# LPD-EPFL/ByzantineMomentum

Measured on AMD Instinct MI355X. Metric: aggregations/sec (Byzantine-robust GAR over n workers x d dims; achieved HBM GB/s per GAR in roofline/per_gar), higher is better.
Workload: dtype f32; 1 GPU; C2 colwise: median + trmean(f=5), n=25, total d=11173962; n_workers=25, f=5, d_total=11173962, d_per_gpu=11173962, byzantine_rows=distinct buffers, row_placement=one torch.empty per row (what a caller of the rules has), parallelism=single GPU, collectives=none

## Files before the change

### byzantinemomentum_amd/csrc/bm_common.h

```cpp
#pragma once
#include <hip/hip_runtime.h>
#include <stdint.h>
#include <utility>
#include "../../include/bm_gar.h"
#include "launch_plan.h"

namespace bm {

struct RowTable {
  const float* p[BM_MAX_ROWS];
  RowTable advanced(int64_t by) const {
    RowTable t = *this;
    advance(t.p, by);
    return t;
  }
};

static inline int hip_code(hipError_t e) { return e == hipSuccess ? 0 : -(int)e; }

#define BM_LAUNCH_CHECK()                      \
  do {                                         \
    hipError_t e__ = hipGetLastError();        \
    if (e__ != hipSuccess) return hip_code(e__); \
  } while (0)

template <int N>
struct MergeExchange {
  static constexpr int kMax = (N < 2) ? 1 : (N * 10);
  struct Table {
    short a[kMax];
    short b[kMax];
    int count;
  };
  static constexpr Table make() {
    Table t{};
    t.count = 0;
    if (N < 2) return t;
    int tt = 0;
    while ((1 << tt) < N) ++tt;
    for (int p = 1 << (tt - 1); p > 0; p /= 2) {
      int q = 1 << (tt - 1), r = 0, d = p;
      while (true) {
        for (int i = 0; i < N - d; ++i)
          if ((i & p) == r) {
            t.a[t.count] = (short)i;
            t.b[t.count] = (short)(i + d);
            ++t.count;
          }
        if (q == p) break;
        d = q - p;
        q /= 2;
        r = p;
      }
    }
    return t;
  }
  static constexpr Table table = make();
};

__device__ __forceinline__ void cmp_exchange(float& a, float& b) {
  float lo, hi;
  asm("v_min_f32 %0, %1, %2" : "=v"(lo) : "v"(a), "v"(b));
  asm("v_max_f32 %0, %1, %2" : "=v"(hi) : "v"(a), "v"(b));
  a = lo;
  b = hi;
}

template <int N, size_t... I>
__device__ __forceinline__ void sort_network_impl(float (&x)[N], std::index_sequence<I...>) {
  (cmp_exchange(x[MergeExchange<N>::table.a[I]], x[MergeExchange<N>::table.b[I]]), ...);
}

template <int N>
__device__ __forceinline__ void sort_network(float (&x)[N]) {
  if constexpr (N >= 2)
    sort_network_impl<N>(x, std::make_index_sequence<MergeExchange<N>::table.count>{});
}

__device__ __forceinline__ float div_small_int(float x, float m, float rm) {
  const float q = x * rm;
  const float r = __builtin_fmaf(-q, m, x);
  const float q1 = __builtin_fmaf(r, rm, q);
  return (q1 == q1) ? q1 : q;
}

template <int VEC>
struct VecLoad;
template <>
struct VecLoad<4> {
  using T = float __attribute__((ext_vector_type(4)));
};
template <>
struct VecLoad<2> {
  using T = float __attribute__((ext_vector_type(2)));
};
template <>
struct VecLoad<1> {
  using T = float;
};

template <int VEC>
__device__ __forceinline__ void load_stream(const float* p, float (&dst)[VEC]) {
  using T = typename VecLoad<VEC>::T;
  const T v = __builtin_nontemporal_load(reinterpret_cast<const T*>(p));
  if constexpr (VEC == 1) {
    dst[0] = v;
  } else {
#pragma unroll
    for (int c = 0; c < VEC; ++c) dst[c] = v[c];
  }
}

template <int VEC>
__device__ __forceinline__ void load_stream_off(const float* base, uint32_t byte_off, float (&dst)[VEC]) {
  load_stream<VEC>(reinterpret_cast<const float*>(reinterpret_cast<const char*>(base) + byte_off), dst);
}

template <int VEC>
__device__ __forceinline__ void store_stream_off(float* base, uint32_t byte_off, const float (&src)[VEC]);

template <int VEC>
__device__ __forceinline__ void store_stream(float* p, const float (&src)[VEC]) {
  using T = typename VecLoad<VEC>::T;
  T v;
  if constexpr (VEC == 1) {
    v = src[0];
  } else {
#pragma unroll
    for (int c = 0; c < VEC; ++c) v[c] = src[c];
  }
  __builtin_nontemporal_store(v, reinterpret_cast<T*>(p));
}

template <int VEC>
__device__ __forceinline__ void store_stream_off(float* base, uint32_t byte_off, const float (&src)[VEC]) {
  store_stream<VEC>(reinterpret_cast<float*>(reinterpret_cast<char*>(base) + byte_off), src);
}

template <int VEC>
__device__ __forceinline__ void store_result(float* p, const float (&src)[VEC]) {
  using T = typename VecLoad<VEC>::T;
  T v;
  if constexpr (VEC == 1) {
    v = src[0];
  } else {
#pragma unroll
    for (int c = 0; c < VEC; ++c) v[c] = src[c];
  }
  *reinterpret_cast<T*>(p) = v;
}
template <int VEC>
__device__ __forceinline__ void store_result_off(float* base, uint32_t byte_off, const float (&src)[VEC]) {
  store_result<VEC>(reinterpret_cast<float*>(reinterpret_cast<char*>(base) + byte_off), src);
}
template <int VEC>
__device__ __forceinline__ void store_result_policy(float* p, const float (&src)[VEC], int nt) {
  if (nt)
    store_stream<VEC>(p, src);
  else
    store_result<VEC>(p, src);
}

constexpr int kColMaxBlocks = 256 * 64;

static inline int lds_opt_in(const void* kernel, size_t dynamic_bytes, size_t static_bytes) {
  if (dynamic_bytes + static_bytes <= 48u * 1024u) return 0;
  return hip_code(hipFuncSetAttribute(kernel, hipFuncAttributeMaxDynamicSharedMemorySize, (int)dynamic_bytes));
}

static inline int compute_units() {
  static int cached[16] = {0};
  int dev = 0;
  if (hipGetDevice(&dev) != hipSuccess || dev < 0 || dev >= 16) dev = 0;
  if (cached[dev] == 0) {
    int cus = 0;
    if (hipDeviceGetAttribute(&cus, hipDeviceAttributeMultiprocessorCount, dev) != hipSuccess || cus <= 0) cus = 256;
    cached[dev] = cus;
  }
  return cached[dev];
}

__device__ __forceinline__ bool arrive_last(int* counter, int total, int* lds_flag) {
  asm volatile("s_waitcnt vmcnt(0)" ::: "memory");
  __syncthreads();
  if (threadIdx.x == 0) {
    __builtin_amdgcn_fence(__ATOMIC_RELEASE, "agent");
    asm volatile("s_waitcnt vmcnt(0)" ::: "memory");
    const int ticket = atomicAdd(counter, 1);
    const int last = (ticket == total - 1) ? 1 : 0;
    if (last) __builtin_amdgcn_fence(__ATOMIC_ACQUIRE, "agent");
    *lds_flag = last;
  }
  __syncthreads();
  return *lds_flag != 0;
}

__device__ __forceinline__ int32_t load_index_coherent(const int32_t* p) {
  return __hip_atomic_load(p, __ATOMIC_RELAXED, __HIP_MEMORY_SCOPE_AGENT);
}

template <int BLOCK>
__device__ __forceinline__ double block_reduce_sum(double v, double* lds ) {
#pragma unroll
  for (int off = 32; off > 0; off >>= 1) v += __shfl_down(v, off, 64);
  const int wave = threadIdx.x >> 6, lane = threadIdx.x & 63;
  if (lane == 0) lds[wave] = v;
  __syncthreads();
  double r = 0.0;
  if (threadIdx.x == 0) {
#pragma unroll
    for (int w = 0; w < BLOCK / 64; ++w) r += lds[w];
  }
  __syncthreads();
  return r;
}

__device__ __forceinline__ float byzantine_coordinate(float avg, float q, float fk, float scale, int attack_kind) {
  const float dir = ((attack_kind & 15) == BM_ATTACK_LITTLE) ? __builtin_sqrtf(q / (fk - 1.0f)) : -avg;
  const float att = dir * scale;
  return (attack_kind & BM_ATTACK_DIRECTION) ? att : avg + att;
}

}

namespace bm {
struct Tuning {
  int col_burst;
  int mean_burst;
  int step_burst;
  int step_stream;
  int pair_mode;
  int pair_planes;
  int pair_dither;
  double pair_tau;
  int study_burst;
  int step_stagger_us;
  int gram_steady;
  int bulyan_short;
  int pair_load_nt;
  int rank_algo;
  int col_wide;
  int brute_budget;
};
const Tuning& tuning();
Tuning& tuning_mutable();
}
```

### byzantinemomentum_amd/csrc/colwise_kernels.h

```cpp
#pragma once
#include "bm_common.h"

namespace bm {

constexpr int kColBlock = 256;

template <int N, int F>
__device__ __forceinline__ float trimmed_sum_static(const float (&x)[N]) {
  float t = 0.0f;
#pragma unroll
  for (int i = F; i < N - F; ++i) t += x[i];
  return t;
}

template <int N>
__device__ __forceinline__ float trimmed_sum(const float (&x)[N], int f) {
  float t = 0.0f;
  switch (f) {
#define BM_TRIM_CASE(F)                                             \
  case F:                                                           \
    if constexpr (2 * (F) < N) t = trimmed_sum_static<N, (F)>(x);   \
    break;
    BM_TRIM_CASE(0) BM_TRIM_CASE(1) BM_TRIM_CASE(2) BM_TRIM_CASE(3) BM_TRIM_CASE(4) BM_TRIM_CASE(5) BM_TRIM_CASE(6)
    BM_TRIM_CASE(7) BM_TRIM_CASE(8) BM_TRIM_CASE(9) BM_TRIM_CASE(10) BM_TRIM_CASE(11) BM_TRIM_CASE(12)
    BM_TRIM_CASE(13) BM_TRIM_CASE(14) BM_TRIM_CASE(15) BM_TRIM_CASE(16) BM_TRIM_CASE(17) BM_TRIM_CASE(18)
    BM_TRIM_CASE(19) BM_TRIM_CASE(20) BM_TRIM_CASE(21) BM_TRIM_CASE(22) BM_TRIM_CASE(23) BM_TRIM_CASE(24)
    BM_TRIM_CASE(25) BM_TRIM_CASE(26) BM_TRIM_CASE(27) BM_TRIM_CASE(28) BM_TRIM_CASE(29) BM_TRIM_CASE(30)
    BM_TRIM_CASE(31)
#undef BM_TRIM_CASE
    default:
      break;
  }
  return t;
}

template <int N, int F>
__device__ __forceinline__ float closest_sum_static(const float (&x)[N], float c) {
  constexpr int M = N - F;
  int s = 0;
#pragma unroll
  for (int t = 0; t < F; ++t) {
    const float dl = __builtin_fabsf(x[t] - c);
    const float dh = __builtin_fabsf(x[t + M] - c);
    s = (dl > dh) ? (t + 1) : s;
  }
  float w = 0.0f;
#pragma unroll
  for (int i = 0; i < N; ++i) {
    if (i < F)
      w += (i >= s) ? x[i] : 0.0f;
    else if (i >= M)
      w += (i < s + M) ? x[i] : 0.0f;
    else
      w += x[i];
  }
  return w;
}

template <int N>
__device__ __forceinline__ float closest_sum(const float (&x)[N], int f, float c) {
  float w = 0.0f;
  switch (f) {
#define BM_CLOSE_CASE(F)                                              \
  case F:                                                             \
    if constexpr (2 * (F) < N) w = closest_sum_static<N, (F)>(x, c);  \
    break;
    BM_CLOSE_CASE(0) BM_CLOSE_CASE(1) BM_CLOSE_CASE(2) BM_CLOSE_CASE(3) BM_CLOSE_CASE(4) BM_CLOSE_CASE(5) BM_CLOSE_CASE(6)
    BM_CLOSE_CASE(7) BM_CLOSE_CASE(8) BM_CLOSE_CASE(9) BM_CLOSE_CASE(10) BM_CLOSE_CASE(11) BM_CLOSE_CASE(12)
    BM_CLOSE_CASE(13) BM_CLOSE_CASE(14) BM_CLOSE_CASE(15) BM_CLOSE_CASE(16) BM_CLOSE_CASE(17) BM_CLOSE_CASE(18)
    BM_CLOSE_CASE(19) BM_CLOSE_CASE(20) BM_CLOSE_CASE(21) BM_CLOSE_CASE(22) BM_CLOSE_CASE(23) BM_CLOSE_CASE(24)
    BM_CLOSE_CASE(25) BM_CLOSE_CASE(26) BM_CLOSE_CASE(27) BM_CLOSE_CASE(28) BM_CLOSE_CASE(29) BM_CLOSE_CASE(30)
    BM_CLOSE_CASE(31)
#undef BM_CLOSE_CASE
    default:
      break;
  }
  return w;
}

template <int N, int OP, int STRIDE = kColBlock>
__device__ __forceinline__ float column_rule(float (&x)[N], int f, float inv_keep, float* ) {
  const float kNaN = __builtin_nanf("");
  const float kInf = __builtin_inff();
  bool has_nan = false;
#pragma unroll
  for (int i = 0; i < N; ++i) has_nan |= (x[i] != x[i]);

  if constexpr (OP == BM_OP_MEDIAN) {
    sort_network<N>(x);
    const float med = x[(N - 1) / 2];
    return has_nan ? kNaN : med;
  } else {
    int nan_count = 0;
    if (__builtin_amdgcn_ballot_w64(has_nan) != 0ull) {
#pragma unroll
      for (int i = 0; i < N; ++i) {
        const bool isn = (x[i] != x[i]);
        nan_count += isn ? 1 : 0;
        x[i] = isn ? kInf : x[i];
      }
    }
    sort_network<N>(x);
    float tsum = 0.0f;
    if constexpr (OP == BM_OP_TRMEAN || OP == BM_OP_PHOCAS) tsum = trimmed_sum<N>(x, f);
    if constexpr (OP == BM_OP_TRMEAN) {
      const float r = div_small_int(tsum, (float)(N - 2 * f), inv_keep);
      return (nan_count > f) ? kNaN : r;
    } else {
      float c;
      if constexpr (OP == BM_OP_PHOCAS) {
        c = div_small_int(tsum, (float)(N - 2 * f), 1.0f / (float)(N - 2 * f));
        if (nan_count > f) c = kNaN;
      } else {
        c = has_nan ? kNaN : x[(N - 1) / 2];
      }
      const int m = N - f;
      const float wsum = closest_sum<N>(x, f, c);
      const float r = div_small_int(wsum, (float)m, inv_keep);
      return (c != c || nan_count > f) ? kNaN : r;
    }
  }
}

template <int N, int OP, int VEC, bool ABLATE_STORE = false>
__global__ __launch_bounds__(kColBlock) void colwise_kernel(RowTable rows, int64_t nvec, int tail,
                                                            int f, float inv_keep, int nt_result,
                                                            float* __restrict__ out) {
  float* const lds = nullptr;
  const uint32_t nv = (uint32_t)nvec;
  const uint32_t stride = gridDim.x * kColBlock;
  for (uint32_t v = blockIdx.x * kColBlock + threadIdx.x; v < nv; v += stride) {
    const uint32_t off = v * (uint32_t)(VEC * sizeof(float));
    float x[VEC][N];
#pragma unroll
    for (int i = 0; i < N; ++i) {
      float t[VEC];
      load_stream_off<VEC>(rows.p[i], off, t);
#pragma unroll
      for (int c = 0; c < VEC; ++c) x[c][i] = t[c];
    }
    float r[VEC];
#pragma unroll
    for (int c = 0; c < VEC; ++c) r[c] = column_rule<N, OP>(x[c], f, inv_keep, lds);
    if constexpr (ABLATE_STORE) {
      if (r[0] == 1.2345678e-30f) store_stream_off<VEC>(out, off, r);
    } else if (nt_result) {
      store_stream_off<VEC>(out, off, r);
    } else {
      store_result_off<VEC>(out, off, r);
    }
  }
  if (VEC > 1 && blockIdx.x == gridDim.x - 1 && (int)threadIdx.x < tail) {
    const int64_t j = nvec * VEC + threadIdx.x;
    float x[N];
#pragma unroll
    for (int i = 0; i < N; ++i) x[i] = rows.p[i][j];
    out[j] = column_rule<N, OP>(x, f, inv_keep, lds);
  }
}

constexpr int kBurstThreads = 1024;
constexpr int kBurstLdsBytes = 160 * 1024;

template <int N, int OP, int VEC>
__global__ __launch_bounds__(kBurstThreads) void colwise_burst_kernel(RowTable rows, int64_t nvec, int tail, int f,
                                                                      float inv_keep, float* __restrict__ out) {
  using V = typename VecLoad<VEC>::T;
  constexpr int kSlots = kBurstLdsBytes / (kBurstThreads * VEC * (int)sizeof(float));
  __shared__ V stage[kSlots * kBurstThreads];
  const uint32_t nv = (uint32_t)nvec, tid = threadIdx.x;
  const uint32_t span = gridDim.x * kBurstThreads;
  const uint32_t iters = (nv + span - 1) / span;
  const uint32_t first = blockIdx.x * kBurstThreads + tid;
  for (uint32_t p0 = 0; p0 < iters; p0 += kSlots) {
    const uint32_t p1 = (p0 + kSlots < iters) ? p0 + kSlots : iters;
    for (uint32_t it = p0; it < p1; ++it) {
      const uint32_t v = it * span + first;
      if (v < nv) {
        const uint32_t off = v * (uint32_t)(VEC * sizeof(float));
        float x[VEC][N];
#pragma unroll
        for (int i = 0; i < N; ++i) {
          float t[VEC];
          load_stream_off<VEC>(rows.p[i], off, t);
#pragma unroll
          for (int c = 0; c < VEC; ++c) x[c][i] = t[c];
        }
        float r[VEC];
#pragma unroll
        for (int c = 0; c < VEC; ++c) r[c] = column_rule<N, OP>(x[c], f, inv_keep, nullptr);
        V packed;
        if constexpr (VEC == 1) {
          packed = r[0];
        } else {
#pragma unroll
          for (int c = 0; c < VEC; ++c) packed[c] = r[c];
        }
        stage[(it - p0) * kBurstThreads + tid] = packed;
      }
    }
    __syncthreads();
    for (uint32_t it = p0; it < p1; ++it) {
      const uint32_t v = it * span + first;
      if (v < nv) {
        const uint32_t off = v * (uint32_t)(VEC * sizeof(float));
        const V packed = stage[(it - p0) * kBurstThreads + tid];
        __builtin_nontemporal_store(packed, reinterpret_cast<V*>(reinterpret_cast<char*>(out) + off));
      }
    }
  }
  if (VEC > 1 && blockIdx.x == gridDim.x - 1 && (int)tid < tail) {
    const int64_t j = nvec * VEC + tid;
    float x[N];
#pragma unroll
    for (int i = 0; i < N; ++i) x[i] = rows.p[i][j];
    out[j] = column_rule<N, OP>(x, f, inv_keep, nullptr);
  }
}

constexpr int kEvalMaxBlocks = 2048;
constexpr Caps kEvalCaps = caps_of(kEvalMaxBlocks);

constexpr int kEvalFinishThreads = 1024;
template <int THREADS>
__global__ __launch_bounds__(THREADS) void eval_finish_kernel(const double* __restrict__ partial, int nparts,
                                                                         double* __restrict__ out) {
  __shared__ double red[THREADS / 64];
  double tot = 0.0;
  for (int b = threadIdx.x; b < nparts; b += THREADS) tot += partial[b];
  const double r = block_reduce_sum<THREADS>(tot, red);
  if (threadIdx.x == 0) out[0] = r;
}


}
```

Before: 5307 agg/s.

## Use min3/med3/max3 sorting networks and compile-time trim count for trmean

Replaces the Batcher merge-exchange sorting network with precomputed tables that mix 3-element sorts (v_min3/v_med3/v_max3) with 2-element compare-exchanges, which cuts the instruction count of the per-column sort for n up to 25. It also dispatches the runtime trim count f to a compile-time constant for trmean, so trimmed sums and the NaN handling specialise fully. The aim is to lower ALU cost in the column-wise median and trmean kernels, at the price of more template instantiations and code size. The hand-built tables must be correct sorting networks.

```diff
diff --git a/byzantinemomentum_amd/csrc/bm_common.h b/byzantinemomentum_amd/csrc/bm_common.h
--- a/byzantinemomentum_amd/csrc/bm_common.h
+++ b/byzantinemomentum_amd/csrc/bm_common.h
@@ -4,6 +4,7 @@
 #include <utility>
 #include "../../include/bm_gar.h"
 #include "launch_plan.h"
+#include "sort_tables.h"
 
 namespace bm {
 
@@ -66,14 +67,39 @@
   b = hi;
 }
 
+__device__ __forceinline__ void sort3(float& a, float& b, float& c) {
+  float lo, mid, hi;
+  asm("v_min3_f32 %0, %1, %2, %3" : "=v"(lo) : "v"(a), "v"(b), "v"(c));
+  asm("v_med3_f32 %0, %1, %2, %3" : "=v"(mid) : "v"(a), "v"(b), "v"(c));
+  asm("v_max3_f32 %0, %1, %2, %3" : "=v"(hi) : "v"(a), "v"(b), "v"(c));
+  a = lo;
+  b = mid;
+  c = hi;
+}
+
 template <int N, size_t... I>
 __device__ __forceinline__ void sort_network_impl(float (&x)[N], std::index_sequence<I...>) {
   (cmp_exchange(x[MergeExchange<N>::table.a[I]], x[MergeExchange<N>::table.b[I]]), ...);
 }
 
+template <int N, size_t I>
+__device__ __forceinline__ void sort_table_op(float (&x)[N]) {
+  constexpr SortOp op = SortTable<N>::ops[I];
+  if constexpr (op.c < 0)
+    cmp_exchange(x[op.a], x[op.b]);
+  else
+    sort3(x[op.a], x[op.b], x[op.c]);
+}
+template <int N, size_t... I>
+__device__ __forceinline__ void sort_table_impl(float (&x)[N], std::index_sequence<I...>) {
+  (sort_table_op<N, I>(x), ...);
+}
+
 template <int N>
 __device__ __forceinline__ void sort_network(float (&x)[N]) {
-  if constexpr (N >= 2)
+  if constexpr (N >= 2 && N <= kSortTableMaxRows)
+    sort_table_impl<N>(x, std::make_index_sequence<SortTable<N>::count>{});
+  else if constexpr (N >= 2)
     sort_network_impl<N>(x, std::make_index_sequence<MergeExchange<N>::table.count>{});
 }
 
diff --git a/byzantinemomentum_amd/csrc/colwise_kernels.h b/byzantinemomentum_amd/csrc/colwise_kernels.h
--- a/byzantinemomentum_amd/csrc/colwise_kernels.h
+++ b/byzantinemomentum_amd/csrc/colwise_kernels.h
@@ -122,6 +122,59 @@
   }
 }
 
+constexpr int kTrimSortMaxRows = kSortTableMaxRows;
+template <int N, int F>
+__device__ __forceinline__ float trmean_column_static(float (&x)[N], float inv_keep) {
+  const float kNaN = __builtin_nanf("");
+  const float kInf = __builtin_inff();
+  bool has_nan = false;
+#pragma unroll
+  for (int i = 0; i < N; ++i) has_nan |= (x[i] != x[i]);
+  int nan_count = 0;
+  if (__builtin_amdgcn_ballot_w64(has_nan) != 0ull) {
+#pragma unroll
+    for (int i = 0; i < N; ++i) {
+      const bool isn = (x[i] != x[i]);
+      nan_count += isn ? 1 : 0;
+      x[i] = isn ? kInf : x[i];
+    }
+  }
+  sort_network<N>(x);
+  const float r = div_small_int(trimmed_sum_static<N, F>(x), (float)(N - 2 * F), inv_keep);
+  return (nan_count > F) ? kNaN : r;
+}
+
+template <int N, int OP, typename Body>
+__device__ __forceinline__ void with_trim_count(int f, Body&& body) {
+  if constexpr (OP == BM_OP_TRMEAN && N <= kTrimSortMaxRows) {
+    static_assert(kTrimSortMaxRows <= 26, "cases for f = 0 .. 12");
+    switch (f) {
+#define BM_TRIM_CASE(F)                                                       \
+  case F:                                                                     \
+    if constexpr (2 * (F) < N) body(std::integral_constant<int, (F)>{});      \
+    break;
+      BM_TRIM_CASE(0) BM_TRIM_CASE(1) BM_TRIM_CASE(2) BM_TRIM_CASE(3) BM_TRIM_CASE(4) BM_TRIM_CASE(5) BM_TRIM_CASE(6)
+      BM_TRIM_CASE(7) BM_TRIM_CASE(8) BM_TRIM_CASE(9) BM_TRIM_CASE(10) BM_TRIM_CASE(11) BM_TRIM_CASE(12)
+#undef BM_TRIM_CASE
+      default:
+        break;
+    }
+  } else {
+    body(std::integral_constant<int, -1>{});
+  }
+}
+
+template <int N, int OP, int VEC, int F>
+__device__ __forceinline__ void column_rules(float (&x)[VEC][N], int f, float inv_keep, float (&r)[VEC]) {
+#pragma unroll
+  for (int c = 0; c < VEC; ++c) {
+    if constexpr (F >= 0)
+      r[c] = trmean_column_static<N, F>(x[c], inv_keep);
+    else
+      r[c] = column_rule<N, OP>(x[c], f, inv_keep, nullptr);
+  }
+}
+
 template <int N, int OP, int VEC, bool ABLATE_STORE = false>
 __global__ __launch_bounds__(kColBlock) void colwise_kernel(RowTable rows, int64_t nvec, int tail,
                                                             int f, float inv_keep, int nt_result,
@@ -129,27 +182,29 @@
   float* const lds = nullptr;
   const uint32_t nv = (uint32_t)nvec;
   const uint32_t stride = gridDim.x * kColBlock;
-  for (uint32_t v = blockIdx.x * kColBlock + threadIdx.x; v < nv; v += stride) {
-    const uint32_t off = v * (uint32_t)(VEC * sizeof(float));
-    float x[VEC][N];
-#pragma unroll
-    for (int i = 0; i < N; ++i) {
-      float t[VEC];
-      load_stream_off<VEC>(rows.p[i], off, t);
-#pragma unroll
-      for (int c = 0; c < VEC; ++c) x[c][i] = t[c];
-    }
-    float r[VEC];
-#pragma unroll
-    for (int c = 0; c < VEC; ++c) r[c] = column_rule<N, OP>(x[c], f, inv_keep, lds);
-    if constexpr (ABLATE_STORE) {
-      if (r[0] == 1.2345678e-30f) store_stream_off<VEC>(out, off, r);
-    } else if (nt_result) {
-      store_stream_off<VEC>(out, off, r);
-    } else {
-      store_result_off<VEC>(out, off, r);
-    }
-  }
+  with_trim_count<N, OP>(f, [&](auto trim) {
+    constexpr int F = decltype(trim)::value;
+    for (uint32_t v = blockIdx.x * kColBlock + threadIdx.x; v < nv; v += stride) {
+      const uint32_t off = v * (uint32_t)(VEC * sizeof(float));
+      float x[VEC][N];
+#pragma unroll
+      for (int i = 0; i < N; ++i) {
+        float t[VEC];
+        load_stream_off<VEC>(rows.p[i], off, t);
+#pragma unroll
+        for (int c = 0; c < VEC; ++c) x[c][i] = t[c];
+      }
+      float r[VEC];
+      column_rules<N, OP, VEC, F>(x, f, inv_keep, r);
+      if constexpr (ABLATE_STORE) {
+        if (r[0] == 1.2345678e-30f) store_stream_off<VEC>(out, off, r);
+      } else if (nt_result) {
+        store_stream_off<VEC>(out, off, r);
+      } else {
+        store_result_off<VEC>(out, off, r);
+      }
+    }
+  });
   if (VEC > 1 && blockIdx.x == gridDim.x - 1 && (int)threadIdx.x < tail) {
     const int64_t j = nvec * VEC + threadIdx.x;
     float x[N];
@@ -172,43 +227,45 @@
   const uint32_t span = gridDim.x * kBurstThreads;
   const uint32_t iters = (nv + span - 1) / span;
   const uint32_t first = blockIdx.x * kBurstThreads + tid;
-  for (uint32_t p0 = 0; p0 < iters; p0 += kSlots) {
-    const uint32_t p1 = (p0 + kSlots < iters) ? p0 + kSlots : iters;
-    for (uint32_t it = p0; it < p1; ++it) {
-      const uint32_t v = it * span + first;
-      if (v < nv) {
-        const uint32_t off = v * (uint32_t)(VEC * sizeof(float));
-        float x[VEC][N];
-#pragma unroll
-        for (int i = 0; i < N; ++i) {
-          float t[VEC];
-          load_stream_off<VEC>(rows.p[i], off, t);
-#pragma unroll
-          for (int c = 0; c < VEC; ++c) x[c][i] = t[c];
+  with_trim_count<N, OP>(f, [&](auto trim) {
+    constexpr int F = decltype(trim)::value;
+    for (uint32_t p0 = 0; p0 < iters; p0 += kSlots) {
+      const uint32_t p1 = (p0 + kSlots < iters) ? p0 + kSlots : iters;
+      for (uint32_t it = p0; it < p1; ++it) {
+        const uint32_t v = it * span + first;
+        if (v < nv) {
+          const uint32_t off = v * (uint32_t)(VEC * sizeof(float));
+          float x[VEC][N];
+#pragma unroll
+          for (int i = 0; i < N; ++i) {
+            float t[VEC];
+            load_stream_off<VEC>(rows.p[i], off, t);
+#pragma unroll
+            for (int c = 0; c < VEC; ++c) x[c][i] = t[c];
+          }
+          float r[VEC];
+          column_rules<N, OP, VEC, F>(x, f, inv_keep, r);
+          V packed;
+          if constexpr (VEC == 1) {
+            packed = r[0];
+          } else {
+#pragma unroll
+            for (int c = 0; c < VEC; ++c) packed[c] = r[c];
+          }
+          stage[(it - p0) * kBurstThreads + tid] = packed;
         }
-        float r[VEC];
-#pragma unroll
-        for (int c = 0; c < VEC; ++c) r[c] = column_rule<N, OP>(x[c], f, inv_keep, nullptr);
-        V packed;
-        if constexpr (VEC == 1) {
-          packed = r[0];
-        } else {
-#pragma unroll
-          for (int c = 0; c < VEC; ++c) packed[c] = r[c];
+      }
+      __syncthreads();
+      for (uint32_t it = p0; it < p1; ++it) {
+        const uint32_t v = it * span + first;
+        if (v < nv) {
+          const uint32_t off = v * (uint32_t)(VEC * sizeof(float));
+          const V packed = stage[(it - p0) * kBurstThreads + tid];
+          __builtin_nontemporal_store(packed, reinterpret_cast<V*>(reinterpret_cast<char*>(out) + off));
         }
-        stage[(it - p0) * kBurstThreads + tid] = packed;
-      }
-    }
-    __syncthreads();
-    for (uint32_t it = p0; it < p1; ++it) {
-      const uint32_t v = it * span + first;
-      if (v < nv) {
-        const uint32_t off = v * (uint32_t)(VEC * sizeof(float));
-        const V packed = stage[(it - p0) * kBurstThreads + tid];
-        __builtin_nontemporal_store(packed, reinterpret_cast<V*>(reinterpret_cast<char*>(out) + off));
-      }
-    }
-  }
+      }
+    }
+  });
   if (VEC > 1 && blockIdx.x == gridDim.x - 1 && (int)tid < tail) {
     const int64_t j = nvec * VEC + tid;
     float x[N];
diff --git a/byzantinemomentum_amd/csrc/sort_tables.h b/byzantinemomentum_amd/csrc/sort_tables.h
--- /dev/null
+++ b/byzantinemomentum_amd/csrc/sort_tables.h
@@ -0,0 +1,331 @@
+#pragma once
+
+namespace bm {
+
+struct SortOp {
+  signed char a, b, c;
+};
+
+constexpr int kSortTableMaxRows = 25;
+
+template <int N>
+struct SortTable;
+
+template <>
+struct SortTable<2> {
+  static constexpr int count = 1;
+  static constexpr SortOp ops[1] = {
+      {0, 1, -1},
+  };
+};
+
+template <>
+struct SortTable<3> {
+  static constexpr int count = 1;
+  static constexpr SortOp ops[1] = {
+      {0, 1, 2},
+  };
+};
+
+template <>
+struct SortTable<4> {
+  static constexpr int count = 4;
+  static constexpr SortOp ops[4] = {
+      {0, 1, 2}, {1, 3, -1}, {0, 1, -1}, {2, 3, -1},
+  };
+};
+
+template <>
+struct SortTable<5> {
+  static constexpr int count = 7;
+  static constexpr SortOp ops[7] = {
+      {0, 2, 4}, {1, 3, -1}, {0, 1, -1}, {2, 3, -1}, {1, 4, -1}, {1, 2, -1}, {3, 4, -1},
+  };
+};
+
+template <>
+struct SortTable<6> {
+  static constexpr int count = 8;
+  static constexpr SortOp ops[8] = {
+      {0, 2, 4}, {1, 3, 5}, {0, 1, -1}, {2, 3, -1}, {4, 5, -1}, {1, 4, -1}, {1, 2, -1}, {3, 4, -1},
+  };
+};
+
+template <>
+struct SortTable<7> {
+  static constexpr int count = 13;
+  static constexpr SortOp ops[13] = {
+      {0, 2, 4}, {1, 3, 5}, {2, 6, -1}, {0, 2, -1}, {4, 6, -1}, {0, 1, -1}, {2, 3, -1}, {4, 5, -1},
+      {1, 4, -1}, {3, 6, -1}, {1, 2, -1}, {3, 4, -1}, {5, 6, -1},
+  };
+};
+
+template <>
+struct SortTable<8> {
+  static constexpr int count = 17;
+  static constexpr SortOp ops[17] = {
+      {0, 2, 4}, {1, 3, 5}, {2, 6, -1}, {3, 7, -1}, {0, 2, -1}, {1, 3, -1}, {4, 6, -1}, {5, 7, -1},
+      {0, 1, -1}, {2, 3, -1}, {4, 5, -1}, {6, 7, -1}, {1, 4, -1}, {3, 6, -1}, {1, 2, -1}, {3, 4, -1},
+      {5, 6, -1},
+  };
+};
+
+template <>
+struct SortTable<9> {
+  static constexpr int count = 13;
+  static constexpr SortOp ops[13] = {
+      {0, 3, 6}, {1, 4, 7}, {2, 5, 8}, {0, 1, 2}, {3, 4, 5}, {6, 7, 8}, {2, 6, -1}, {1, 3, -1},
+      {4, 6, -1}, {5, 7, -1}, {2, 4, -1}, {2, 3, -1}, {5, 6, -1},
+  };
+};
+
+template <>
+struct SortTable<10> {
+  static constexpr int count = 22;
+  static constexpr SortOp ops[22] = {
+      {0, 3, 6}, {1, 4, 7}, {2, 5, 8}, {0, 1, 2}, {3, 4, 5}, {6, 7, 8}, {1, 9, -1}, {2, 6, -1},
+      {5, 9, -1}, {1, 3, -1}, {4, 6, -1}, {5, 7, -1}, {2, 4, -1}, {3, 5, -1}, {7, 9, -1}, {0, 1, -1},
+      {2, 3, -1}, {4, 5, -1}, {6, 7, -1}, {8, 9, -1}, {3, 4, -1}, {5, 6, -1},
+  };
+};
+
+template <>
+struct SortTable<11> {
+  static constexpr int count = 29;
+  static constexpr SortOp ops[29] = {
+      {0, 4, 8}, {1, 5, 9}, {2, 6, 10}, {0, 1, 2}, {4, 5, 6}, {8, 9, 10}, {3, 7, -1}, {1, 3, -1},
+      {5, 7, -1}, {2, 8, -1}, {3, 9, -1}, {2, 4, -1}, {3, 5, -1}, {6, 8, -1}, {7, 9, -1}, {0, 1, -1},
+      {2, 3, -1}, {4, 5, -1}, {6, 7, -1}, {8, 9, -1}, {1, 4, -1}, {3, 6, -1}, {5, 8, -1}, {7, 10, -1},
+      {1, 2, -1}, {3, 4, -1}, {5, 6, -1}, {7, 8, -1}, {9, 10, -1},
+  };
+};
+
+template <>
+struct SortTable<12> {
+  static constexpr int count = 31;
+  static constexpr SortOp ops[31] = {
+      {0, 4, 8}, {1, 5, 9}, {2, 6, 10}, {3, 7, 11}, {0, 1, 2}, {4, 5, 6}, {8, 9, 10}, {1, 3, -1},
+      {5, 7, -1}, {9, 11, -1}, {2, 8, -1}, {3, 9, -1}, {2, 4, -1}, {3, 5, -1}, {6, 8, -1}, {7, 9, -1},
+      {0, 1, -1}, {2, 3, -1}, {4, 5, -1}, {6, 7, -1}, {8, 9, -1}, {10, 11, -1}, {1, 4, -1}, {3, 6, -1},
+      {5, 8, -1}, {7, 10, -1}, {1, 2, -1}, {3, 4, -1}, {5, 6, -1}, {7, 8, -1}, {9, 10, -1},
+  };
+};
+
+template <>
+struct SortTable<13> {
+  static constexpr int count = 38;
+  static constexpr SortOp ops[38] = {
+      {0, 4, 8}, {1, 5, 9}, {2, 6, 10}, {3, 7, 11}, {0, 1, 2}, {4, 5, 6}, {8, 9, 10}, {4, 12, -1},
+      {0, 4, -1}, {8, 12, -1}, {1, 3, -1}, {5, 7, -1}, {9, 11, -1}, {2, 8, -1}, {3, 9, -1}, {6, 12, -1},
+      {2, 4, -1}, {3, 5, -1}, {6, 8, -1}, {7, 9, -1}, {10, 12, -1}, {0, 1, -1}, {2, 3, -1}, {4, 5, -1},
+      {6, 7, -1}, {8, 9, -1}, {10, 11, -1}, {1, 4, -1}, {3, 6, -1}, {5, 8, -1}, {7, 10, -1}, {9, 12, -1},
+      {1, 2, -1}, {3, 4, -1}, {5, 6, -1}, {7, 8, -1}, {9, 10, -1}, {11, 12, -1},
+  };
+};
+
+template <>
+struct SortTable<14> {
+  static constexpr int count = 44;
+  static constexpr SortOp ops[44] = {
+      {0, 4, 8}, {1, 5, 9}, {2, 6, 10}, {3, 7, 11}, {0, 1, 2}, {4, 5, 6}, {8, 9, 10}, {4, 12, -1},
+      {5, 13, -1}, {0, 4, -1}, {1, 5, -1}, {8, 12, -1}, {9, 13, -1}, {1, 3, -1}, {5, 7, -1}, {9, 11, -1},
+      {2, 8, -1}, {3, 9, -1}, {6, 12, -1}, {7, 13, -1}, {2, 4, -1}, {3, 5, -1}, {6, 8, -1}, {7, 9, -1},
+      {10, 12, -1}, {11, 13, -1}, {0, 1, -1}, {2, 3, -1}, {4, 5, -1}, {6, 7, -1}, {8, 9, -1}, {10, 11, -1},
+      {12, 13, -1}, {1, 4, -1}, {3, 6, -1}, {5, 8, -1}, {7, 10, -1}, {9, 12, -1}, {1, 2, -1}, {3, 4, -1},
+      {5, 6, -1}, {7, 8, -1}, {9, 10, -1}, {11, 12, -1},
+  };
+};
+
+template <>
+struct SortTable<15> {
+  static constexpr int count = 50;
+  static constexpr SortOp ops[50] = {
+      {0, 4, 8}, {1, 5, 9}, {2, 6, 10}, {3, 7, 11}, {0, 1, 2}, {4, 5, 6}, {8, 9, 10}, {12, 13, 14},
+      {4, 12, -1}, {5, 13, -1}, {6, 14, -1}, {0, 4, -1}, {1, 5, -1}, {2, 6, -1}, {8, 12, -1}, {9, 13, -1},
+      {10, 14, -1}, {1, 3, -1}, {5, 7, -1}, {9, 11, -1}, {2, 8, -1}, {3, 9, -1}, {6, 12, -1}, {7, 13, -1},
+      {2, 4, -1}, {3, 5, -1}, {6, 8, -1}, {7, 9, -1}, {10, 12, -1}, {11, 13, -1}, {0, 1, -1}, {2, 3, -1},
+      {4, 5, -1}, {6, 7, -1}, {8, 9, -1}, {10, 11, -1}, {12, 13, -1}, {1, 4, -1}, {3, 6, -1}, {5, 8, -1},
+      {7, 10, -1}, {9, 12, -1}, {11, 14, -1}, {1, 2, -1}, {3, 4, -1}, {5, 6, -1}, {7, 8, -1}, {9, 10, -1},
+      {11, 12, -1}, {13, 14, -1},
+  };
+};
+
+template <>
+struct SortTable<16> {
+  static constexpr int count = 55;
+  static constexpr SortOp ops[55] = {
+      {0, 4, 8}, {1, 5, 9}, {2, 6, 10}, {3, 7, 11}, {0, 1, 2}, {4, 5, 6}, {8, 9, 10}, {12, 13, 14},
+      {4, 12, -1}, {5, 13, -1}, {6, 14, -1}, {7, 15, -1}, {0, 4, -1}, {1, 5, -1}, {2, 6, -1}, {3, 7, -1},
+      {8, 12, -1}, {9, 13, -1}, {10, 14, -1}, {11, 15, -1}, {1, 3, -1}, {5, 7, -1}, {9, 11, -1}, {13, 15, -1},
+      {2, 8, -1}, {3, 9, -1}, {6, 12, -1}, {7, 13, -1}, {2, 4, -1}, {3, 5, -1}, {6, 8, -1}, {7, 9, -1},
+      {10, 12, -1}, {11, 13, -1}, {0, 1, -1}, {2, 3, -1}, {4, 5, -1}, {6, 7, -1}, {8, 9, -1}, {10, 11, -1},
+      {12, 13, -1}, {14, 15, -1}, {1, 4, -1}, {3, 6, -1}, {5, 8, -1}, {7, 10, -1}, {9, 12, -1}, {11, 14, -1},
+      {1, 2, -1}, {3, 4, -1}, {5, 6, -1}, {7, 8, -1}, {9, 10, -1}, {11, 12, -1}, {13, 14, -1},
+  };
+};
+
+template <>
+struct SortTable<17> {
+  static constexpr int count = 58;
+  static constexpr SortOp ops[58] = {
+      {0, 6, 12}, {1, 7, 13}, {2, 8, 14}, {3, 9, 15}, {4, 10, 16}, {0, 2, 4}, {1, 3, 5}, {6, 8, 10},
+      {7, 9, 11}, {12, 14, 16}, {4, 12, -1}, {5, 13, -1}, {2, 6, -1}, {3, 7, -1}, {8, 12, -1}, {9, 13, -1},
+      {10, 14, -1}, {11, 15, -1}, {4, 8, -1}, {5, 9, -1}, {7, 11, -1}, {1, 3, -1}, {4, 6, -1}, {5, 7, -1},
+      {9, 11, -1}, {13, 15, -1}, {7, 9, -1}, {10, 12, -1}, {11, 13, -1}, {0, 1, -1}, {2, 3, -1}, {4, 5, -1},
+      {6, 7, -1}, {8, 9, -1}, {10, 11, -1}, {12, 13, -1}, {14, 15, -1}, {1, 16, -1}, {1, 8, -1}, {3, 10, -1},
+      {5, 12, -1}, {7, 14, -1}, {9, 16, -1}, {1, 4, -1}, {3, 6, -1}, {5, 8, -1}, {7, 10, -1}, {9, 12, -1},
+      {11, 14, -1}, {13, 16, -1}, {1, 2, -1}, {3, 4, -1}, {5, 6, -1}, {7, 8, -1}, {9, 10, -1}, {11, 12, -1},
+      {13, 14, -1}, {15, 16, -1},
+  };
+};
+
+template <>
+struct SortTable<18> {
+  static constexpr int count = 56;
+  static constexpr SortOp ops[56] = {
+      {0, 6, 12}, {1, 7, 13}, {2, 8, 14}, {3, 9, 15}, {4, 10, 16}, {5, 11, 17}, {0, 2, 4}, {1, 3, 5},
+      {6, 8, 10}, {7, 9, 11}, {12, 14, 16}, {13, 15, 17}, {4, 12, -1}, {5, 13, -1}, {2, 6, -1}, {3, 7, -1},
+      {8, 12, -1}, {9, 13, -1}, {10, 14, -1}, {11, 15, -1}, {4, 8, -1}, {5, 9, -1}, {4, 6, -1}, {5, 7, -1},
+      {10, 12, -1}, {11, 13, -1}, {0, 1, -1}, {2, 3, -1}, {4, 5, -1}, {6, 7, -1}, {8, 9, -1}, {10, 11, -1},
+      {12, 13, -1}, {14, 15, -1}, {16, 17, -1}, {1, 16, -1}, {1, 8, -1}, {3, 10, -1}, {5, 12, -1}, {7, 14, -1},
+      {9, 16, -1}, {1, 4, -1}, {3, 6, -1}, {5, 8, -1}, {7, 10, -1}, {9, 12, -1}, {11, 14, -1}, {13, 16, -1},
+      {1, 2, -1}, {3, 4, -1}, {5, 6, -1}, {7, 8, -1}, {9, 10, -1}, {11, 12, -1}, {13, 14, -1}, {15, 16, -1},
+  };
+};
+
+template <>
+struct SortTable<19> {
+  static constexpr int count = 69;
+  static constexpr SortOp ops[69] = {
+      {0, 6, 12}, {1, 7, 13}, {2, 8, 14}, {3, 9, 15}, {4, 10, 16}, {5, 11, 17}, {0, 2, 4}, {1, 3, 5},
+      {6, 8, 10}, {7, 9, 11}, {12, 14, 16}, {13, 15, 17}, {2, 18, -1}, {4, 12, -1}, {5, 13, -1}, {10, 18, -1},
+      {2, 6, -1}, {3, 7, -1}, {8, 12, -1}, {9, 13, -1}, {10, 14, -1}, {11, 15, -1}, {4, 8, -1}, {5, 9, -1},
+      {6, 10, -1}, {14, 18, -1}, {0, 2, -1}, {4, 6, -1}, {5, 7, -1}, {8, 10, -1}, {12, 14, -1}, {16, 18, -1},
+      {6, 8, -1}, {10, 12, -1}, {11, 13, -1}, {0, 1, -1}, {2, 3, -1}, {4, 5, -1}, {6, 7, -1}, {8, 9, -1},
+      {10, 11, -1}, {12, 13, -1}, {14, 15, -1}, {16, 17, -1}, {1, 16, -1}, {3, 18, -1}, {1, 8, -1}, {3, 10, -1},
+      {5, 12, -1}, {7, 14, -1}, {9, 16, -1}, {11, 18, -1}, {1, 4, -1}, {3, 6, -1}, {5, 8, -1}, {7, 10, -1},
+      {9, 12, -1}, {11, 14, -1}, {13, 16, -1}, {15, 18, -1}, {1, 2, -1}, {3, 4, -1}, {5, 6, -1}, {7, 8, -1},
+      {9, 10, -1}, {11, 12, -1}, {13, 14, -1}, {15, 16, -1}, {17, 18, -1},
+  };
+};
+
+template <>
+struct SortTable<20> {
+  static constexpr int count = 79;
+  static constexpr SortOp ops[79] = {
+      {0, 6, 12}, {1, 7, 13}, {2, 8, 14}, {3, 9, 15}, {4, 10, 16}, {5, 11, 17}, {0, 2, 4}, {1, 3, 5},
+      {6, 8, 10}, {7, 9, 11}, {12, 14, 16}, {13, 15, 17}, {2, 18, -1}, {3, 19, -1}, {4, 12, -1}, {5, 13, -1},
+      {10, 18, -1}, {11, 19, -1}, {2, 6, -1}, {3, 7, -1}, {8, 12, -1}, {9, 13, -1}, {10, 14, -1}, {11, 15, -1},
+      {4, 8, -1}, {5, 9, -1}, {6, 10, -1}, {7, 11, -1}, {14, 18, -1}, {15, 19, -1}, {0, 2, -1}, {1, 3, -1},
+      {4, 6, -1}, {5, 7, -1}, {8, 10, -1}, {9, 11, -1}, {12, 14, -1}, {13, 15, -1}, {16, 18, -1}, {17, 19, -1},
+      {6, 8, -1}, {7, 9, -1}, {10, 12, -1}, {11, 13, -1}, {0, 1, -1}, {2, 3, -1}, {4, 5, -1}, {6, 7, -1},
+      {8, 9, -1}, {10, 11, -1}, {12, 13, -1}, {14, 15, -1}, {16, 17, -1}, {18, 19, -1}, {1, 16, -1}, {3, 18, -1},
+      {1, 8, -1}, {3, 10, -1}, {5, 12, -1}, {7, 14, -1}, {9, 16, -1}, {11, 18, -1}, {1, 4, -1}, {3, 6, -1},
+      {5, 8, -1}, {7, 10, -1}, {9, 12, -1}, {11, 14, -1}, {13, 16, -1}, {15, 18, -1}, {1, 2, -1}, {3, 4, -1},
+      {5, 6, -1}, {7, 8, -1}, {9, 10, -1}, {11, 12, -1}, {13, 14, -1}, {15, 16, -1}, {17, 18, -1},
+  };
+};
+
+template <>
+struct SortTable<21> {
+  static constexpr int count = 92;
+  static constexpr SortOp ops[92] = {
+      {0, 6, 12}, {1, 7, 13}, {2, 8, 14}, {3, 9, 15}, {4, 10, 16}, {5, 11, 17}, {0, 2, 4}, {1, 3, 5},
+      {6, 8, 10}, {7, 9, 11}, {12, 14, 16}, {13, 15, 17}, {2, 18, -1}, {3, 19, -1}, {4, 20, -1}, {4, 12, -1},
+      {5, 13, -1}, {10, 18, -1}, {11, 19, -1}, {12, 20, -1}, {0, 4, -1}, {2, 6, -1}, {3, 7, -1}, {8, 12, -1},
+      {9, 13, -1}, {10, 14, -1}, {11, 15, -1}, {16, 20, -1}, {4, 8, -1}, {5, 9, -1}, {6, 10, -1}, {7, 11, -1},
+      {12, 16, -1}, {14, 18, -1}, {15, 19, -1}, {0, 2, -1}, {1, 3, -1}, {4, 6, -1}, {5, 7, -1}, {8, 10, -1},
+      {9, 11, -1}, {12, 14, -1}, {13, 15, -1}, {16, 18, -1}, {17, 19, -1}, {10, 16, -1}, {2, 4, -1}, {6, 8, -1},
+      {7, 9, -1}, {10, 12, -1}, {11, 13, -1}, {14, 16, -1}, {18, 20, -1}, {0, 1, -1}, {2, 3, -1}, {4, 5, -1},
+      {6, 7, -1}, {8, 9, -1}, {10, 11, -1}, {12, 13, -1}, {14, 15, -1}, {16, 17, -1}, {18, 19, -1}, {1, 16, -1},
+      {3, 18, -1}, {5, 20, -1}, {1, 8, -1}, {3, 10, -1}, {5, 12, -1}, {7, 14, -1}, {9, 16, -1}, {11, 18, -1},
+      {13, 20, -1}, {1, 4, -1}, {3, 6, -1}, {5, 8, -1}, {7, 10, -1}, {9, 12, -1}, {11, 14, -1}, {13, 16, -1},
+      {15, 18, -1}, {17, 20, -1}, {1, 2, -1}, {3, 4, -1}, {5, 6, -1}, {7, 8, -1}, {9, 10, -1}, {11, 12, -1},
+      {13, 14, -1}, {15, 16, -1}, {17, 18, -1}, {19, 20, -1},
+  };
+};
+
+template <>
+struct SortTable<22> {
+  static constexpr int count = 98;
+  static constexpr SortOp ops[98] = {
+      {0, 8, 16}, {1, 9, 17}, {2, 10, 18}, {3, 11, 19}, {4, 12, 20}, {5, 13, 21}, {0, 2, 4}, {1, 3, 5},
+      {8, 10, 12}, {9, 11, 13}, {16, 18, 20}, {17, 19, 21}, {6, 14, -1}, {7, 15, -1}, {2, 6, -1}, {3, 7, -1},
+      {10, 14, -1}, {11, 15, -1}, {4, 16, -1}, {5, 17, -1}, {6, 18, -1}, {7, 19, -1}, {4, 8, -1}, {5, 9, -1},
+      {6, 10, -1}, {7, 11, -1}, {12, 16, -1}, {13, 17, -1}, {14, 18, -1}, {15, 19, -1}, {0, 2, -1}, {1, 3, -1},
+      {4, 6, -1}, {5, 7, -1}, {8, 10, -1}, {9, 11, -1}, {12, 14, -1}, {13, 15, -1}, {16, 18, -1}, {17, 19, -1},
+      {2, 8, -1}, {3, 9, -1}, {6, 12, -1}, {7, 13, -1}, {10, 16, -1}, {11, 17, -1}, {14, 20, -1}, {15, 21, -1},
+      {2, 4, -1}, {3, 5, -1}, {6, 8, -1}, {7, 9, -1}, {10, 12, -1}, {11, 13, -1}, {14, 16, -1}, {15, 17, -1},
+      {18, 20, -1}, {19, 21, -1}, {0, 1, -1}, {2, 3, -1}, {4, 5, -1}, {6, 7, -1}, {8, 9, -1}, {10, 11, -1},
+      {12, 13, -1}, {14, 15, -1}, {16, 17, -1}, {18, 19, -1}, {20, 21, -1}, {1, 16, -1}, {3, 18, -1}, {5, 20, -1},
+      {1, 8, -1}, {3, 10, -1}, {5, 12, -1}, {7, 14, -1}, {9, 16, -1}, {11, 18, -1}, {13, 20, -1}, {1, 4, -1},
+      {3, 6, -1}, {5, 8, -1}, {7, 10, -1}, {9, 12, -1}, {11, 14, -1}, {13, 16, -1}, {15, 18, -1}, {17, 20, -1},
+      {1, 2, -1}, {3, 4, -1}, {5, 6, -1}, {7, 8, -1}, {9, 10, -1}, {11, 12, -1}, {13, 14, -1}, {15, 16, -1},
+      {17, 18, -1}, {19, 20, -1},
+  };
+};
+
+template <>
+struct SortTable<23> {
+  static constexpr int count = 104;
+  static constexpr SortOp ops[104] = {
+      {0, 8, 16}, {1, 9, 17}, {2, 10, 18}, {3, 11, 19}, {4, 12, 20}, {5, 13, 21}, {6, 14, 22}, {0, 2, 4},
+      {1, 3, 5}, {8, 10, 12}, {9, 11, 13}, {16, 18, 20}, {17, 19, 21}, {7, 15, -1}, {2, 6, -1}, {3, 7, -1},
+      {10, 14, -1}, {11, 15, -1}, {18, 22, -1}, {4, 16, -1}, {5, 17, -1}, {6, 18, -1}, {7, 19, -1}, {4, 8, -1},
+      {5, 9, -1}, {6, 10, -1}, {7, 11, -1}, {12, 16, -1}, {13, 17, -1}, {14, 18, -1}, {15, 19, -1}, {0, 2, -1},
+      {1, 3, -1}, {4, 6, -1}, {5, 7, -1}, {8, 10, -1}, {9, 11, -1}, {12, 14, -1}, {13, 15, -1}, {16, 18, -1},
+      {17, 19, -1}, {20, 22, -1}, {2, 8, -1}, {3, 9, -1}, {6, 12, -1}, {7, 13, -1}, {10, 16, -1}, {11, 17, -1},
+      {14, 20, -1}, {15, 21, -1}, {2, 4, -1}, {3, 5, -1}, {6, 8, -1}, {7, 9, -1}, {10, 12, -1}, {11, 13, -1},
+      {14, 16, -1}, {15, 17, -1}, {18, 20, -1}, {19, 21, -1}, {0, 1, -1}, {2, 3, -1}, {4, 5, -1}, {6, 7, -1},
+      {8, 9, -1}, {10, 11, -1}, {12, 13, -1}, {14, 15, -1}, {16, 17, -1}, {18, 19, -1}, {20, 21, -1}, {1, 16, -1},
+      {3, 18, -1}, {5, 20, -1}, {7, 22, -1}, {1, 8, -1}, {3, 10, -1}, {5, 12, -1}, {7, 14, -1}, {9, 16, -1},
+      {11, 18, -1}, {13, 20, -1}, {15, 22, -1}, {1, 4, -1}, {3, 6, -1}, {5, 8, -1}, {7, 10, -1}, {9, 12, -1},
+      {11, 14, -1}, {13, 16, -1}, {15, 18, -1}, {17, 20, -1}, {19, 22, -1}, {1, 2, -1}, {3, 4, -1}, {5, 6, -1},
+      {7, 8, -1}, {9, 10, -1}, {11, 12, -1}, {13, 14, -1}, {15, 16, -1}, {17, 18, -1}, {19, 20, -1}, {21, 22, -1},
+  };
+};
+
+template <>
+struct SortTable<24> {
+  static constexpr int count = 107;
+  static constexpr SortOp ops[107] = {
+      {0, 8, 16}, {1, 9, 17}, {2, 10, 18}, {3, 11, 19}, {4, 12, 20}, {5, 13, 21}, {6, 14, 22}, {7, 15, 23},
+      {0, 2, 4}, {1, 3, 5}, {8, 10, 12}, {9, 11, 13}, {16, 18, 20}, {17, 19, 21}, {2, 6, -1}, {3, 7, -1},
+      {10, 14, -1}, {11, 15, -1}, {18, 22, -1}, {19, 23, -1}, {4, 16, -1}, {5, 17, -1}, {6, 18, -1}, {7, 19, -1},
+      {4, 8, -1}, {5, 9, -1}, {6, 10, -1}, {7, 11, -1}, {12, 16, -1}, {13, 17, -1}, {14, 18, -1}, {15, 19, -1},
+      {0, 2, -1}, {1, 3, -1}, {4, 6, -1}, {5, 7, -1}, {8, 10, -1}, {9, 11, -1}, {12, 14, -1}, {13, 15, -1},
+      {16, 18, -1}, {17, 19, -1}, {20, 22, -1}, {21, 23, -1}, {2, 8, -1}, {3, 9, -1}, {6, 12, -1}, {7, 13, -1},
+      {10, 16, -1}, {11, 17, -1}, {14, 20, -1}, {15, 21, -1}, {2, 4, -1}, {3, 5, -1}, {6, 8, -1}, {7, 9, -1},
+      {10, 12, -1}, {11, 13, -1}, {14, 16, -1}, {15, 17, -1}, {18, 20, -1}, {19, 21, -1}, {0, 1, -1}, {2, 3, -1},
+      {4, 5, -1}, {6, 7, -1}, {8, 9, -1}, {10, 11, -1}, {12, 13, -1}, {14, 15, -1}, {16, 17, -1}, {18, 19, -1},
+      {20, 21, -1}, {22, 23, -1}, {1, 16, -1}, {3, 18, -1}, {5, 20, -1}, {7, 22, -1}, {1, 8, -1}, {3, 10, -1},
+      {5, 12, -1}, {7, 14, -1}, {9, 16, -1}, {11, 18, -1}, {13, 20, -1}, {15, 22, -1}, {1, 4, -1}, {3, 6, -1},
+      {5, 8, -1}, {7, 10, -1}, {9, 12, -1}, {11, 14, -1}, {13, 16, -1}, {15, 18, -1}, {17, 20, -1}, {19, 22, -1},
+      {1, 2, -1}, {3, 4, -1}, {5, 6, -1}, {7, 8, -1}, {9, 10, -1}, {11, 12, -1}, {13, 14, -1}, {15, 16, -1},
+      {17, 18, -1}, {19, 20, -1}, {21, 22, -1},
+  };
+};
+
+template <>
+struct SortTable<25> {
+  static constexpr int count = 118;
+  static constexpr SortOp ops[118] = {
+      {0, 8, 16}, {1, 9, 17}, {2, 10, 18}, {3, 11, 19}, {4, 12, 20}, {5, 13, 21}, {6, 14, 22}, {7, 15, 23},
+      {0, 2, 4}, {1, 3, 5}, {8, 10, 12}, {9, 11, 13}, {16, 18, 20}, {17, 19, 21}, {8, 24, -1}, {0, 8, -1},
+      {16, 24, -1}, {2, 6, -1}, {3, 7, -1}, {10, 14, -1}, {11, 15, -1}, {18, 22, -1}, {19, 23, -1}, {4, 16, -1},
+      {5, 17, -1}, {6, 18, -1}, {7, 19, -1}, {12, 24, -1}, {4, 8, -1}, {5, 9, -1}, {6, 10, -1}, {7, 11, -1},
+      {12, 16, -1}, {13, 17, -1}, {14, 18, -1}, {15, 19, -1}, {20, 24, -1}, {0, 2, -1}, {1, 3, -1}, {4, 6, -1},
+      {5, 7, -1}, {8, 10, -1}, {9, 11, -1}, {12, 14, -1}, {13, 15, -1}, {16, 18, -1}, {17, 19, -1}, {20, 22, -1},
+      {21, 23, -1}, {2, 8, -1}, {3, 9, -1}, {6, 12, -1}, {7, 13, -1}, {10, 16, -1}, {11, 17, -1}, {14, 20, -1},
+      {15, 21, -1}, {18, 24, -1}, {2, 4, -1}, {3, 5, -1}, {6, 8, -1}, {7, 9, -1}, {10, 12, -1}, {11, 13, -1},
+      {14, 16, -1}, {15, 17, -1}, {18, 20, -1}, {19, 21, -1}, {22, 24, -1}, {0, 1, -1}, {2, 3, -1}, {4, 5, -1},
+      {6, 7, -1}, {8, 9, -1}, {10, 11, -1}, {12, 13, -1}, {14, 15, -1}, {16, 17, -1}, {18, 19, -1}, {20, 21, -1},
+      {22, 23, -1}, {1, 16, -1}, {3, 18, -1}, {5, 20, -1}, {7, 22, -1}, {9, 24, -1}, {1, 8, -1}, {3, 10, -1},
+      {5, 12, -1}, {7, 14, -1}, {9, 16, -1}, {11, 18, -1}, {13, 20, -1}, {15, 22, -1}, {17, 24, -1}, {1, 4, -1},
+      {3, 6, -1}, {5, 8, -1}, {7, 10, -1}, {9, 12, -1}, {11, 14, -1}, {13, 16, -1}, {15, 18, -1}, {17, 20, -1},
+      {19, 22, -1}, {21, 24, -1}, {1, 2, -1}, {3, 4, -1}, {5, 6, -1}, {7, 8, -1}, {9, 10, -1}, {11, 12, -1},
+      {13, 14, -1}, {15, 16, -1}, {17, 18, -1}, {19, 20, -1}, {21, 22, -1}, {23, 24, -1},
+  };
+};
+
+}
```

Result: faster. 5361 agg/s (median of 6 runs) (+1.0%).
